# CycloneBoy/pdf_table

Hardware: AMD Instinct MI355X
Metric: pages/s (higher is better)
Workload: dtype bf16

## Files before the change

### pdf_table_amd/csrc/lore_kernels.hip

```cpp
#include <stdio.h>
#include <stdlib.h>

#include "common.h"

namespace PT_FMT_NS {

typedef __attribute__((ext_vector_type(4))) uint32_t u32x4;
typedef __attribute__((ext_vector_type(2))) uint32_t u32x2;

namespace {

__device__ __forceinline__ float bf2f(uint32_t b) { return a16_to_f32(b); }
__device__ __forceinline__ uint32_t f2bf(float f) { return f32_to_a16(f); }

__device__ __forceinline__ void load8(const bf16_t* p, int lo_off, int split, float* v) {
  const u32x4 h = *reinterpret_cast<const u32x4*>(p);
  const uint32_t hw[4] = {h.x, h.y, h.z, h.w};
#pragma unroll
  for (int k = 0; k < 8; ++k) v[k] = bf2f((k & 1) ? (hw[k >> 1] >> 16) : (hw[k >> 1] & 0xFFFFu));
  if (split) {
    const u32x4 l = *reinterpret_cast<const u32x4*>(p + lo_off);
    const uint32_t lw[4] = {l.x, l.y, l.z, l.w};
#pragma unroll
    for (int k = 0; k < 8; ++k) v[k] += bf2f((k & 1) ? (lw[k >> 1] >> 16) : (lw[k >> 1] & 0xFFFFu));
// ... 241 lines not shown
  const int y = i / W, x = i - y * W;
  const pt_tsr_table tb = tabs[t];
  auto sat = [](double v) { return (long long)fmin(fmax(rint(v), -2147483648.0), 2147483647.0); };
  const long long adelta = sat(tb.minv[0] * x * 1024.0), bdelta = sat(tb.minv[3] * x * 1024.0);
  const long long X0 = sat((tb.minv[1] * y + tb.minv[2]) * 1024.0) + 16, Y0 = sat((tb.minv[4] * y + tb.minv[5]) * 1024.0) + 16;
  const long long X = (X0 + adelta) >> 5, Y = (Y0 + bdelta) >> 5;
  long long sx = X >> 5, sy = Y >> 5;
  sx = sx < -32768 ? -32768 : (sx > 32767 ? 32767 : sx);
  sy = sy < -32768 ? -32768 : (sy > 32767 ? 32767 : sy);
  const int ax = (int)(X & 31), ay = (int)(Y & 31);
  const int wt[4] = {(32 - ay) * (32 - ax) * 32, (32 - ay) * ax * 32, ay * (32 - ax) * 32, ay * ax * 32};
  int acc[3] = {0, 0, 0};
  const uint8_t* pg = pages + (size_t)tb.page * ph * pw * 3;
#pragma unroll
  for (int k = 0; k < 4; ++k) {
    const long long yy = sy + (k >> 1), xx = sx + (k & 1);
    if (yy < 0 || yy >= tb.crop_h || xx < 0 || xx >= tb.crop_w) continue;
    const long long py = tb.y0 + yy, px = tb.x0 + xx;
    if (py < 0 || py >= ph || px < 0 || px >= pw) continue;
    const uint8_t* s = pg + ((size_t)py * pw + px) * 3;
    acc[0] += s[0] * wt[k]; acc[1] += s[1] * wt[k]; acc[2] += s[2] * wt[k];
  }
  float v[3];
#pragma unroll
  for (int c = 0; c < 3; ++c) {
    const int sc = bgr ? 2 - c : c;
    int u = (acc[sc] + (1 << 14)) >> 15;
    u = u < 0 ? 0 : (u > 255 ? 255 : u);
    v[c] = lut[c * 256 + u];
  }
  bf16_t* o = out + ((size_t)t * H * W + i) * (split ? 8 : 4);
  uint32_t hb[3];
#pragma unroll
  for (int c = 0; c < 3; ++c) { hb[c] = f2bf(v[c]); o[c] = (bf16_t)hb[c]; }
  o[3] = 0;
  if (split) {
#pragma unroll
    for (int c = 0; c < 3; ++c) o[4 + c] = (bf16_t)f2bf(v[c] - bf2f(hb[c]));
    o[7] = 0;
  }
}

typedef __attribute__((ext_vector_type(8))) __bf16 dbf16x8;
typedef __attribute__((ext_vector_type(16))) float df32x16;
typedef __attribute__((ext_vector_type(2))) float df2;
__device__ __forceinline__ uint32_t pack_df2(df2 v) { return pack_a16x2(v.x, v.y); }
__device__ __forceinline__ df2 unpack_df2(uint32_t pk) { return df2{a16lo_f32(pk), a16hi_f32(pk)}; }

template <int SPLIT, int NB>
__global__ __launch_bounds__(256, (SPLIT || NB > 64) ? 2 : 4) void dcn_fused_kernel(const bf16_t* __restrict__ x, const float* __restrict__ om,
                                                            const bf16_t* __restrict__ w, const float* __restrict__ bias,
                                                            bf16_t* __restrict__ out, long long npix, int H, int W, int C,
                                                            int N, int relu) {
#pragma clang fp contract(fast)
  a16_kernel_enter();
  constexpr int ROW = 80;
  constexpr int NP = SPLIT ? 2 : 1;
  constexpr int NT = NB / 32;
  __shared__ __attribute__((aligned(16))) char s_a[NP][128 * ROW];
  __shared__ __attribute__((aligned(16))) char s_w[NP][NB * ROW];
  const int tid = threadIdx.x, lane = tid & 63, wave = tid >> 6;
  const int lx = lane & 31, q = lane >> 5;
  const long long p0 = (long long)blockIdx.x * 128;
  const int n0 = blockIdx.y * NB;
  const int cs = SPLIT ? 2 * C : C;
  const int nslice = C >> 5, nk = 9 * nslice;
  const int gp = tid & 127, gh = tid >> 7;
  long long pix = p0 + gp;
  const bool live = pix < npix;
  if (!live) pix = npix - 1;
  const int xw = (int)(pix % W), yh = (int)((pix / W) % H);
  const bf16_t* xb = x + (size_t)(pix / ((long long)W * H)) * H * W * cs;
  const float* omp = om + pix * 32;
  constexpr int WPIECES = NB * 4 / 256;
  const bf16_t* wbase = w + (size_t)(n0 >> 6) * (SPLIT ? 3 : 1) * nk * (64 * 32);

  df32x16 acc[NT];
#pragma unroll
  for (int t = 0; t < NT; ++t)
#pragma unroll
    for (int r = 0; r < 16; ++r) acc[t][r] = 0.f;

  int coff[4];
  float cwt[4], mask = 0.f;
  u32x4 rc[NP][4][2];
  u32x4 rw[NP][WPIECES];

  auto geometry = [&](int tap) {
    const float off_h = omp[2 * tap], off_w = omp[2 * tap + 1];
    mask = 1.f / (1.f + expf(-omp[18 + tap]));
    const float h_im = (float)(yh - 1 + tap / 3) + off_h;
    const float w_im = (float)(xw - 1 + tap % 3) + off_w;
#pragma unroll
    for (int k = 0; k < 4; ++k) { coff[k] = -1; cwt[k] = 0.f; }
    if (h_im > -1.f && w_im > -1.f && h_im < (float)H && w_im < (float)W) {
      const float hf = floorf(h_im), wf = floorf(w_im);
      const int h_low = (int)hf, w_low = (int)wf, h_high = h_low + 1, w_high = w_low + 1;
      const float lh = h_im - hf, lw = w_im - wf, hh = 1.f - lh, hw = 1.f - lw;
      cwt[0] = hh * hw; cwt[1] = hh * lw; cwt[2] = lh * hw; cwt[3] = lh * lw;
      if (h_low >= 0 && w_low >= 0) coff[0] = (h_low * W + w_low) * cs;
      if (h_low >= 0 && w_high <= W - 1) coff[1] = (h_low * W + w_high) * cs;
      if (h_high <= H - 1 && w_low >= 0) coff[2] = (h_high * W + w_low) * cs;
      if (h_high <= H - 1 && w_high <= W - 1) coff[3] = (h_high * W + w_high) * cs;
    }
  };
  auto prefetch = [&](int kc) {
    const int tap = kc / nslice, sl = kc - tap * nslice;
    if (sl == 0) geometry(tap);
    const int ch = sl * 32 + gh * 16;
#pragma unroll
    for (int k = 0; k < 4; ++k) {
      const u32x4 z = {0u, 0u, 0u, 0u};
#pragma unroll
      for (int pp = 0; pp < NP; ++pp) {
        rc[pp][k][0] = z; rc[pp][k][1] = z;
        if (coff[k] >= 0) {
          const bf16_t* sp = xb + coff[k] + ch + pp * C;
          rc[pp][k][0] = *reinterpret_cast<const u32x4*>(sp);
          rc[pp][k][1] = *reinterpret_cast<const u32x4*>(sp + 8);
        }
      }
    }
#pragma unroll
    for (int j = 0; j < WPIECES; ++j) {
      const int idx = tid + j * 256;
      const int row = idx >> 2, part = idx & 3;
      const bf16_t* wc = wbase + (size_t)(row >> 6) * (SPLIT ? 3 : 1) * nk * (64 * 32) + (size_t)kc * (64 * 32) + (row & 63) * 32 + part * 8;
      rw[0][j] = *reinterpret_cast<const u32x4*>(wc);
      if (SPLIT) rw[1][j] = *reinterpret_cast<const u32x4*>(wc + (size_t)2 * nk * (64 * 32));
    }
  };
  auto commit = [&]() {
    const df2 w0 = {cwt[0], cwt[0]}, w1 = {cwt[1], cwt[1]}, w2 = {cwt[2], cwt[2]}, w3 = {cwt[3], cwt[3]}, mk = {mask, mask};
    uint32_t oh[8], ol[8];
#pragma unroll
    for (int hgrp = 0; hgrp < 2; ++hgrp) {
#pragma unroll
      for (int e2 = 0; e2 < 4; ++e2) {
        df2 c[4];
#pragma unroll
        for (int k = 0; k < 4; ++k) {
          const uint32_t u = e2 == 0 ? rc[0][k][hgrp].x : e2 == 1 ? rc[0][k][hgrp].y : e2 == 2 ? rc[0][k][hgrp].z : rc[0][k][hgrp].w;
          c[k] = df2{a16lo_f32(u), a16hi_f32(u)};
          if (SPLIT) {
            const uint32_t ul = e2 == 0 ? rc[NP - 1][k][hgrp].x : e2 == 1 ? rc[NP - 1][k][hgrp].y
                                : e2 == 2 ? rc[NP - 1][k][hgrp].z : rc[NP - 1][k][hgrp].w;
            c[k] += df2{a16lo_f32(ul), a16hi_f32(ul)};
          }
        }
        df2 v = w0 * c[0];
        v = w1 * c[1] + v;
        v = w2 * c[2] + v;
        v = w3 * c[3] + v;
        v = v * mk;
        const uint32_t hb = pack_df2(v);
        oh[hgrp * 4 + e2] = hb;
        if (SPLIT) ol[hgrp * 4 + e2] = pack_df2(v - unpack_df2(hb));
      }
    }
    char* ap = s_a[0] + gp * ROW + gh * 32;
    *reinterpret_cast<u32x4*>(ap) = u32x4{oh[0], oh[1], oh[2], oh[3]};
    *reinterpret_cast<u32x4*>(ap + 16) = u32x4{oh[4], oh[5], oh[6], oh[7]};
    if (SPLIT) {
      char* al = s_a[NP - 1] + gp * ROW + gh * 32;
      *reinterpret_cast<u32x4*>(al) = u32x4{ol[0], ol[1], ol[2], ol[3]};
      *reinterpret_cast<u32x4*>(al + 16) = u32x4{ol[4], ol[5], ol[6], ol[7]};
    }
#pragma unroll
    for (int j = 0; j < WPIECES; ++j) {
      const int idx = tid + j * 256;
#pragma unroll
      for (int pp = 0; pp < NP; ++pp) *reinterpret_cast<u32x4*>(s_w[pp] + (idx >> 2) * ROW + (idx & 3) * 16) = rw[pp][j];
    }
  };

  const char* a_rd = s_a[0] + (wave * 32 + lx) * ROW + q * 16;
  const char* b_rd = s_w[0] + lx * ROW + q * 16;
  constexpr int A_PLANE = 128 * ROW, W_PLANE = NB * ROW;
  prefetch(0);
  for (int kc = 0; kc < nk; ++kc) {
    __syncthreads();
    commit();
    __syncthreads();
    if (kc + 1 < nk) prefetch(kc + 1);
#pragma unroll
    for (int kk = 0; kk < 2; ++kk) {
      const dbf16x8 ah = *reinterpret_cast<const dbf16x8*>(a_rd + kk * 32);
      dbf16x8 al;
      if (SPLIT) al = *reinterpret_cast<const dbf16x8*>(a_rd + A_PLANE + kk * 32);
#pragma unroll
      for (int t = 0; t < NT; ++t) {
        const dbf16x8 bh = *reinterpret_cast<const dbf16x8*>(b_rd + t * 32 * ROW + kk * 32);
        acc[t] = mfma_32x32x16_a16(ah, bh, acc[t]);
        if (SPLIT) {
          acc[t] = mfma_32x32x16_a16(al, bh, acc[t]);
          const dbf16x8 bl = *reinterpret_cast<const dbf16x8*>(b_rd + W_PLANE + t * 32 * ROW + kk * 32);
          acc[t] = mfma_32x32x16_a16(ah, bl, acc[t]);
        }
      }
    }
  }
  const int ocs = SPLIT ? 2 * N : N;
#pragma unroll
  for (int t = 0; t < NT; ++t) {
    const int n = n0 + t * 32 + lx;
    const float bv = bias[n];
#pragma unroll
    for (int r = 0; r < 16; ++r) {
      const long long op = p0 + wave * 32 + (r & 3) + 8 * (r >> 2) + 4 * q;
      if (op >= npix) continue;
      float v = acc[t][r] + bv;
      if (relu) v = fmaxf(v, 0.f);
      const uint32_t hb = f2bf(v);
      out[(size_t)op * ocs + n] = (bf16_t)hb;
      if (SPLIT) out[(size_t)op * ocs + N + n] = (bf16_t)f2bf(v - bf2f(hb));
    }
  }
}

#ifndef PT_DCN_ABL
#define PT_DCN_ABL 0
#endif
template <int NB, int NTHR, int SPLIT = 0, int EARLY = 0, int OMF = 0>
__global__ __launch_bounds__(NTHR, SPLIT ? (NB == 128 ? 1 : 2) : NTHR / 128) void dcn_fused64_kernel(const bf16_t* __restrict__ x, const float* __restrict__ om,
                                                              const bf16_t* __restrict__ w, const float* __restrict__ bias,
                                                              bf16_t* __restrict__ out, long long npix, int H, int W,
                                                              int C, int N, int relu, const bf16_t* __restrict__ omw = nullptr,
                                                              const float* __restrict__ omb = nullptr) {
#pragma clang fp contract(fast)
  a16_kernel_enter();
  constexpr int ROW = 144;
  constexpr int IT = 1024 / NTHR;
  constexpr int PSTEP = NTHR / 8;
  constexpr int WP = NB * 8 / NTHR;
  constexpr int NT = NB * 8 / NTHR;
  constexpr int NP = SPLIT ? 2 : 1;
  __shared__ __attribute__((aligned(16))) unsigned s_goff[128 * 9][4];
  __shared__ __attribute__((aligned(16))) float s_gwt[128 * 9][4];
  __shared__ __attribute__((aligned(16))) char s_ab[NP * (128 * ROW + NB * ROW)];
  static_assert(128 * ROW + NB * ROW >= 128 * 28 * 4, "operand images must cover the staged offset/mask rows");
  constexpr int A_PLANE = 128 * ROW, W_PLANE = NB * ROW;
  char* s_a = s_ab;
  char* s_w = s_ab + NP * A_PLANE;
  float* s_om = reinterpret_cast<float*>(s_ab);
  const int tid = threadIdx.x, lane = tid & 63, wave = tid >> 6;
  const int lx = lane & 31, q = lane >> 5;
  const int tiles_x = (W + 15) >> 4, tiles_y = (H + 7) >> 3;
  int Lb = blockIdx.x;
  const int nblk = blockIdx.y;
  const int tx0 = (Lb % tiles_x) * 16;
  Lb /= tiles_x;
  const int ty0 = (Lb % tiles_y) * 8;
  const long long img0 = (long long)(Lb / tiles_y) * H * W;
  auto locate = [&](int pl, int& y, int& xq) -> bool {
    y = ty0 + (pl >> 4);
    xq = tx0 + (pl & 15);
    const bool ok = y < H && xq < W;
    y = y < H ? y : H - 1;
    xq = xq < W ? xq : W - 1;
    return ok;
  };
  const int n0 = nblk * NB;
  const int nss = C >> 6, nst = 9 * nss, nk = 9 * (C >> 5);
  const int cs = SPLIT ? 2 * C : C;
  const int piece = tid & 7, prow = tid >> 3;
  const char* xmap = reinterpret_cast<const char*>(x + (size_t)img0 * cs);
  if constexpr (OMF) {
    constexpr int HP = 180, HROW = 80;
    constexpr int HIT = (HP * 4 + NTHR - 1) / NTHR;
    constexpr int NG = NTHR / 256;
    static_assert(sizeof(s_goff) >= HP * HROW && sizeof(s_gwt) >= HP * HROW, "a halo buffer must fit each table's space");
    char* s_h = reinterpret_cast<char*>(&s_goff[0][0]);
    char* s_h2 = reinterpret_cast<char*>(&s_gwt[0][0]);
    const int nch = (SPLIT ? 3 : 1) * (C >> 5);
    const int grp = wave >> 2, mt_o = wave & 3;
    const int t_lo = NG == 2 ? (grp ? 5 : 0) : 0, t_hi = NG == 2 ? (grp ? 9 : 5) : 9;
    u32x4 hreg[HIT];
    auto halo_load = [&](int kc) {
      int c0 = kc * 32;
      if (SPLIT && kc >= 2 * (C >> 5)) c0 -= 2 * C;
#pragma unroll
      for (int j = 0; j < HIT; ++j) {
        const int i = tid + j * NTHR;
        const int hp = i >> 2, hy = hp / 18, hx = hp - hy * 18;
        const int y = ty0 - 1 + hy, xq = tx0 - 1 + hx;
        u32x4 v = {0u, 0u, 0u, 0u};
        if (i < HP * 4 && (unsigned)y < (unsigned)H && (unsigned)xq < (unsigned)W)
          v = *reinterpret_cast<const u32x4*>(xmap + ((size_t)y * W + xq) * (2 * cs) + (size_t)c0 * 2 + (i & 3) * 16);
        hreg[j] = v;
      }
    };
    auto halo_store = [&](char* buf) {
#pragma unroll
      for (int j = 0; j < HIT; ++j) {
        const int i = tid + j * NTHR;
        if (i < HP * 4) *reinterpret_cast<u32x4*>(buf + (i >> 2) * HROW + (i & 3) * 16) = hreg[j];
      }
    };
    df32x16 oacc;
#pragma unroll
    for (int r = 0; r < 16; ++r) oacc[r] = 0.f;
    const int pl_o = mt_o * 32 + lx;
    const int a_off = ((pl_o >> 4) * 18 + (pl_o & 15)) * HROW + q * 16;
    const bf16_t* wl = omw + (size_t)lx * 32 + q * 8;
    constexpr int NTAP = NG == 2 ? 5 : 9;
    dbf16x8 bfr[NTAP][2];
    auto load_b = [&](int kc, int t) {
      const bf16_t* wt = wl + ((size_t)kc * 9 + (t_lo + t)) * 2048;
      bfr[t][0] = *reinterpret_cast<const dbf16x8*>(wt);
      bfr[t][1] = *reinterpret_cast<const dbf16x8*>(wt + 16);
    };
    halo_load(0);
#pragma unroll
    for (int t = 0; t < NTAP; ++t)
      if (t_lo + t < t_hi) load_b(0, t);
    for (int kc = 0; kc < nch; ++kc) {
      char* buf = (kc & 1) ? s_h2 : s_h;
      halo_store(buf);
      if (kc + 1 < nch) halo_load(kc + 1);
      __syncthreads();
#pragma unroll
      for (int t = 0; t < NTAP; ++t) {
        const int tap = t_lo + t;
        if (tap < t_hi) {
          const char* ap = buf + a_off + ((tap / 3) * 18 + (tap % 3)) * HROW;
          const dbf16x8 a0 = *reinterpret_cast<const dbf16x8*>(ap);
          const dbf16x8 a1 = *reinterpret_cast<const dbf16x8*>(ap + 32);
          oacc = mfma_32x32x16_a16(a0, bfr[t][0], oacc);
          oacc = mfma_32x32x16_a16(a1, bfr[t][1], oacc);
          if (kc + 1 < nch) load_b(kc + 1, t);
        }
      }
    }
    if (wave < 4 && lx < 27) {
      const float bo = omb[lx];
#pragma unroll
      for (int r = 0; r < 16; ++r) s_om[(mt_o * 32 + (r & 3) + 8 * (r >> 2) + 4 * q) * 28 + lx] = oacc[r] + bo;
    }
    if (NG == 2) {
      __syncthreads();
      if (wave >= 4 && lx < 27) {
#pragma unroll
        for (int r = 0; r < 16; ++r) s_om[(mt_o * 32 + (r & 3) + 8 * (r >> 2) + 4 * q) * 28 + lx] += oacc[r];
      }
    }
  } else {
    for (int i = tid; i < 128 * 7; i += NTHR) {
      int y, xq;
      locate(i / 7, y, xq);
      const long long pix = img0 + (long long)y * W + xq;
      *reinterpret_cast<float4*>(s_om + (i / 7) * 28 + (i % 7) * 4) = *reinterpret_cast<const float4*>(om + pix * 32 + (i % 7) * 4);
    }
  }
  __syncthreads();
  for (int i = tid; i < 128 * 9; i += NTHR) {
    const int pl = i / 9, tap = i - pl * 9;
    int yh, xw;
    locate(pl, yh, xw);
    const float* o = s_om + pl * 28;
    const float off_h = o[2 * tap], off_w = o[2 * tap + 1];
    const float gm = 1.f / (1.f + expf(-o[18 + tap]));
    const float h_im = (float)(yh - 1 + tap / 3) + off_h;
    const float w_im = (float)(xw - 1 + tap % 3) + off_w;
    unsigned co[4] = {0u, 0u, 0u, 0u};
    float cw[4] = {0.f, 0.f, 0.f, 0.f};
    if (h_im > -1.f && w_im > -1.f && h_im < (float)H && w_im < (float)W) {
      const float hf = floorf(h_im), wf = floorf(w_im);
      const int h_low = (int)hf, w_low = (int)wf, h_high = h_low + 1, w_high = w_low + 1;
      const float lh = h_im - hf, lw = w_im - wf, hh = 1.f - lh, hw = 1.f - lw;
      if (h_low >= 0 && w_low >= 0) { co[0] = (unsigned)(h_low * W + w_low) * (unsigned)(2 * cs); cw[0] = hh * hw * gm; }
      if (h_low >= 0 && w_high <= W - 1) { co[1] = (unsigned)(h_low * W + w_high) * (unsigned)(2 * cs); cw[1] = hh * lw * gm; }
      if (h_high <= H - 1 && w_low >= 0) { co[2] = (unsigned)(h_high * W + w_low) * (unsigned)(2 * cs); cw[2] = lh * hw * gm; }
      if (h_high <= H - 1 && w_high <= W - 1) { co[3] = (unsigned)(h_high * W + w_high) * (unsigned)(2 * cs); cw[3] = lh * lw * gm; }
    }
    *reinterpret_cast<uint4*>(s_goff[i]) = make_uint4(co[0], co[1], co[2], co[3]);
    *reinterpret_cast<float4*>(s_gwt[i]) = make_float4(cw[0], cw[1], cw[2], cw[3]);
  }
  __syncthreads();
  const bf16_t* wbase = w + (size_t)(n0 >> 6) * (SPLIT ? 3 : 1) * nk * (64 * 32);

  df32x16 acc[NT];
#pragma unroll
  for (int t = 0; t < NT; ++t)
#pragma unroll
    for (int r = 0; r < 16; ++r) acc[t][r] = 0.f;

  unsigned coff[IT][4];
  float cwt[IT][4];
  u32x4 rc[IT][4], rcl[SPLIT ? IT : 1][4];
  u32x4 rw[WP], rwl[SPLIT ? WP : 1];

  auto geometry = [&](int tap) {
#pragma unroll
    for (int j = 0; j < IT; ++j) {
      const int gi = (prow + PSTEP * j) * 9 + tap;
      const uint4 o = *reinterpret_cast<const uint4*>(s_goff[gi]);
      const float4 wv = *reinterpret_cast<const float4*>(s_gwt[gi]);
      coff[j][0] = o.x + piece * 16; coff[j][1] = o.y + piece * 16; coff[j][2] = o.z + piece * 16; coff[j][3] = o.w + piece * 16;
      cwt[j][0] = wv.x; cwt[j][1] = wv.y; cwt[j][2] = wv.z; cwt[j][3] = wv.w;
    }
  };
  auto prefetch = [&](int st) {
    const int tap = st / nss, ss = st - tap * nss;
    if (ss == 0) geometry(tap);
    const char* xs = xmap + ss * 128;
#pragma unroll
    for (int j = 0; j < IT; ++j)
#pragma unroll
      for (int k = 0; k < 4; ++k) {
#if PT_DCN_ABL == 1
        rc[j][k] = u32x4{coff[j][k], 0u, 0u, 0u};
#else
        rc[j][k] = *reinterpret_cast<const u32x4*>(xs + coff[j][k]);
#endif
        if (SPLIT) rcl[j][k] = *reinterpret_cast<const u32x4*>(xs + 2 * C + coff[j][k]);
      }
    const int kc = tap * (C >> 5) + 2 * ss;
#pragma unroll
    for (int j = 0; j < WP; ++j) {
      const int idx = tid + j * NTHR;
      const int row = idx >> 3, pc = idx & 7;
      const bf16_t* wsrc = wbase + (size_t)(row >> 6) * (SPLIT ? 3 : 1) * nk * (64 * 32) + (size_t)(kc + (pc >> 2)) * (64 * 32) +
                           (row & 63) * 32 + (pc & 3) * 8;
      rw[j] = *reinterpret_cast<const u32x4*>(wsrc);
      if (SPLIT) rwl[j] = *reinterpret_cast<const u32x4*>(wsrc + (size_t)2 * nk * (64 * 32));
    }
  };
  auto commit = [&]() {
#pragma unroll
    for (int j = 0; j < IT; ++j) {
#if PT_DCN_ABL == 2
      *reinterpret_cast<u32x4*>(s_a + (prow + PSTEP * j) * ROW + piece * 16) = rc[j][0] ^ rc[j][1] ^ rc[j][2] ^ rc[j][3];
      continue;
#endif
      const df2 w0 = {cwt[j][0], cwt[j][0]}, w1 = {cwt[j][1], cwt[j][1]}, w2 = {cwt[j][2], cwt[j][2]},
                w3 = {cwt[j][3], cwt[j][3]};
      uint32_t o[4], ol[4];
#pragma unroll
      for (int e2 = 0; e2 < 4; ++e2) {
        if constexpr (PT_A16_HAS_MIX_BLEND && !SPLIT) {
          o[e2] = a16_blend4(rc[j][0][e2], rc[j][1][e2], rc[j][2][e2], rc[j][3][e2], cwt[j][0], cwt[j][1], cwt[j][2], cwt[j][3]);
          continue;
        }
        df2 c[4];
#pragma unroll
        for (int k = 0; k < 4; ++k) {
          const uint32_t u = e2 == 0 ? rc[j][k].x : e2 == 1 ? rc[j][k].y : e2 == 2 ? rc[j][k].z : rc[j][k].w;
          c[k] = df2{a16lo_f32(u), a16hi_f32(u)};
          if (SPLIT) {
            const uint32_t ul = e2 == 0 ? rcl[j][k].x : e2 == 1 ? rcl[j][k].y : e2 == 2 ? rcl[j][k].z : rcl[j][k].w;
            c[k] += df2{a16lo_f32(ul), a16hi_f32(ul)};
          }
        }
        df2 v = w0 * c[0];
        v = w1 * c[1] + v;
        v = w2 * c[2] + v;
        v = w3 * c[3] + v;
        const uint32_t hb = pack_df2(v);
        o[e2] = hb;
        if (SPLIT) ol[e2] = pack_df2(v - unpack_df2(hb));
      }
      *reinterpret_cast<u32x4*>(s_a + (prow + PSTEP * j) * ROW + piece * 16) = u32x4{o[0], o[1], o[2], o[3]};
      if (SPLIT) *reinterpret_cast<u32x4*>(s_a + A_PLANE + (prow + PSTEP * j) * ROW + piece * 16) = u32x4{ol[0], ol[1], ol[2], ol[3]};
    }
#pragma unroll
    for (int j = 0; j < WP; ++j) {
      const int idx = tid + j * NTHR;
      *reinterpret_cast<u32x4*>(s_w + (idx >> 3) * ROW + (idx & 7) * 16) = rw[j];
      if (SPLIT) *reinterpret_cast<u32x4*>(s_w + W_PLANE + (idx >> 3) * ROW + (idx & 7) * 16) = rwl[j];
    }
  };

  const int mt = wave & 3, ct0 = (wave >> 2) * NT;
  const char* a_rd = s_a + (mt * 32 + lx) * ROW + q * 16;
  const char* b_rd = s_w + (ct0 * 32 + lx) * ROW + q * 16;
  auto product = [&]() {
#pragma unroll
    for (int kk = 0; kk < 4; ++kk) {
      const dbf16x8 a = *reinterpret_cast<const dbf16x8*>(a_rd + kk * 32);
      dbf16x8 al;
      if (SPLIT) al = *reinterpret_cast<const dbf16x8*>(a_rd + A_PLANE + kk * 32);
#pragma unroll
      for (int t = 0; t < NT; ++t) {
        const dbf16x8 b = *reinterpret_cast<const dbf16x8*>(b_rd + t * 32 * ROW + kk * 32);
#if PT_DCN_ABL == 3
        if (kk == 0 && t == 0)
#endif
        acc[t] = mfma_32x32x16_a16(b, a, acc[t]);
        if (SPLIT) {
          acc[t] = mfma_32x32x16_a16(b, al, acc[t]);
          const dbf16x8 bl = *reinterpret_cast<const dbf16x8*>(b_rd + W_PLANE + t * 32 * ROW + kk * 32);
          acc[t] = mfma_32x32x16_a16(bl, a, acc[t]);
        }
      }
    }
  };
  if constexpr (EARLY && !SPLIT) {
    prefetch(0);
    for (int st = 0; st < nst; ++st) {
      const bool more = st + 1 < nst;
      const int tap_n = (st + 1) / nss, ss_n = (st + 1) - tap_n * nss;
      const char* xs_n = xmap + ss_n * 128;
      __syncthreads();
#pragma unroll
      for (int j = 0; j < IT; ++j) {
        const df2 w0 = {cwt[j][0], cwt[j][0]}, w1 = {cwt[j][1], cwt[j][1]}, w2 = {cwt[j][2], cwt[j][2]}, w3 = {cwt[j][3], cwt[j][3]};
        uint32_t o[4];
#pragma unroll
        for (int e2 = 0; e2 < 4; ++e2) {
          if constexpr (PT_A16_HAS_MIX_BLEND) {
            o[e2] = a16_blend4(rc[j][0][e2], rc[j][1][e2], rc[j][2][e2], rc[j][3][e2], cwt[j][0], cwt[j][1], cwt[j][2], cwt[j][3]);
            continue;
          }
          df2 c[4];
#pragma unroll
          for (int k = 0; k < 4; ++k) {
            const uint32_t u = e2 == 0 ? rc[j][k].x : e2 == 1 ? rc[j][k].y : e2 == 2 ? rc[j][k].z : rc[j][k].w;
            c[k] = df2{a16lo_f32(u), a16hi_f32(u)};
          }
          df2 v = w0 * c[0];
          v = w1 * c[1] + v;
          v = w2 * c[2] + v;
          v = w3 * c[3] + v;
          o[e2] = pack_df2(v);
        }
        *reinterpret_cast<u32x4*>(s_a + (prow + PSTEP * j) * ROW + piece * 16) = u32x4{o[0], o[1], o[2], o[3]};
        if (more) {
          if (ss_n == 0) {
            const int gi = (prow + PSTEP * j) * 9 + tap_n;
            const uint4 og = *reinterpret_cast<const uint4*>(s_goff[gi]);
            const float4 wv = *reinterpret_cast<const float4*>(s_gwt[gi]);
            coff[j][0] = og.x + piece * 16; coff[j][1] = og.y + piece * 16; coff[j][2] = og.z + piece * 16; coff[j][3] = og.w + piece * 16;
            cwt[j][0] = wv.x; cwt[j][1] = wv.y; cwt[j][2] = wv.z; cwt[j][3] = wv.w;
          }
#pragma unroll
          for (int k = 0; k < 4; ++k) rc[j][k] = *reinterpret_cast<const u32x4*>(xs_n + coff[j][k]);
        }
      }
#pragma unroll
      for (int j = 0; j < WP; ++j) {
        const int idx = tid + j * NTHR;
        *reinterpret_cast<u32x4*>(s_w + (idx >> 3) * ROW + (idx & 7) * 16) = rw[j];
      }
      if (more) {
        const int kc = tap_n * (C >> 5) + 2 * ss_n;
#pragma unroll
        for (int j = 0; j < WP; ++j) {
          const int idx = tid + j * NTHR;
          const int row = idx >> 3, pc = idx & 7;
          rw[j] = *reinterpret_cast<const u32x4*>(wbase + (size_t)(row >> 6) * nk * (64 * 32) + (size_t)(kc + (pc >> 2)) * (64 * 32) + (row & 63) * 32 + (pc & 3) * 8);
        }
      }
      __syncthreads();
      product();
    }
  } else {
    prefetch(0);
    for (int st = 0; st < nst; ++st) {
      __syncthreads();
      commit();
      __syncthreads();
      if (st + 1 < nst) prefetch(st + 1);
      product();
    }
  }
  int y, xq;
  if (locate(mt * 32 + lx, y, xq)) {
    bf16_t* op = out + (size_t)(img0 + (long long)y * W + xq) * (SPLIT ? 2 * N : N) + n0 + ct0 * 32;
#pragma unroll
    for (int t = 0; t < NT; ++t)
#pragma unroll
      for (int rg = 0; rg < 4; ++rg) {
        const int ch = t * 32 + 8 * rg + 4 * q;
        const float4 bs = *reinterpret_cast<const float4*>(bias + n0 + ct0 * 32 + ch);
        float v[4] = {acc[t][rg * 4 + 0] + bs.x, acc[t][rg * 4 + 1] + bs.y, acc[t][rg * 4 + 2] + bs.z, acc[t][rg * 4 + 3] + bs.w};
        if (relu) {
#pragma unroll
          for (int j = 0; j < 4; ++j) v[j] = fmaxf(v[j], 0.f);
        }
        const uint32_t h0 = f2bf(v[0]), h1 = f2bf(v[1]), h2 = f2bf(v[2]), h3 = f2bf(v[3]);
        *reinterpret_cast<uint2*>(op + ch) = make_uint2(h0 | (h1 << 16), h2 | (h3 << 16));
        if (SPLIT)
          *reinterpret_cast<uint2*>(op + N + ch) = make_uint2(f2bf(v[0] - bf2f(h0)) | (f2bf(v[1] - bf2f(h1)) << 16),
                                                               f2bf(v[2] - bf2f(h2)) | (f2bf(v[3] - bf2f(h3)) << 16));
      }
  }
}

#ifndef PT_DCN_MABL
#define PT_DCN_MABL 0
#endif
#ifndef PT_DCN_RING64
#define PT_DCN_RING64 4
#endif
template <int NB, int RING>
struct DcnMfmaSmem {
  static constexpr int BYTES = 128 * 9 * 24 + 2 * NB * 128 + 8 * RING * 1024;
};
template <int NB, int RING>
__global__ __launch_bounds__(512, (NB == 64 && RING == 4) ? 2 : 1) void dcn_mfma_kernel(const bf16_t* __restrict__ x, const float* __restrict__ om,
                                                                            const bf16_t* __restrict__ w, const float* __restrict__ bias,
                                                                            bf16_t* __restrict__ out, long long npix, int H, int W, int C,
                                                                            int N, int relu) {
#pragma clang fp contract(fast)
  a16_kernel_enter();
  static_assert(RING == 4 || RING == 8, "ring slots must divide the eight steps of a stage");
  constexpr int NT = NB / 32;
  constexpr int WP = NB / 64;
  constexpr int D = RING - 1;
  constexpr int GOFF_BYTES = 128 * 9 * 16, GW_BYTES = 128 * 9 * 8, W_BYTES = NB * 128;
  extern __shared__ __attribute__((aligned(16))) char smem[];
  char* s_goff = smem;
  char* s_gw = smem + GOFF_BYTES;
  char* s_w = s_gw + GW_BYTES;
  char* s_ring = s_w + 2 * W_BYTES;
  float* s_om = reinterpret_cast<float*>(s_ring);
  static_assert(8 * RING * 1024 >= 128 * 28 * 4, "ring must cover the staged offset / mask rows");
  const int tid = threadIdx.x, lane = tid & 63, wave = tid >> 6;
  const int lx = lane & 31, q = lane >> 5;
  const int pt = wave & 3, hh = wave >> 2;
  const int tiles_x = (W + 15) >> 4, tiles_y = (H + 7) >> 3;
  int Lb = blockIdx.x;
  const int tx0 = (Lb % tiles_x) * 16;
  Lb /= tiles_x;
  const int ty0 = (Lb % tiles_y) * 8;
  const long long img0 = (long long)(Lb / tiles_y) * H * W;
  auto locate = [&](int pl, int& y, int& xq) -> bool {
    y = ty0 + (pl >> 4);
    xq = tx0 + (pl & 15);
    const bool ok = y < H && xq < W;
    y = y < H ? y : H - 1;
    xq = xq < W ? xq : W - 1;
    return ok;
  };
  const int n0 = blockIdx.y * NB;
  const int nss = C >> 6, nst = 9 * nss, nk = 9 * (C >> 5);
// ... 989 lines not shown
```

Baseline: 779.5.

## Stage offset-conv weights through shared memory instead of per-wave register prefetch

Offset-conv weights for each channel chunk are now loaded cooperatively by the whole block into registers, stored into a padded LDS region that reuses the operand-image buffer, and read from LDS by each wave for the MFMA taps. Before, every wave fetched its own B fragments from global memory into a large per-tap register array. The aim is to cut redundant global loads and register pressure. In exchange it adds an extra barrier per chunk and a trailing one, and uses more LDS traffic.

```diff
diff --git a/pdf_table_amd/csrc/lore_kernels.hip b/pdf_table_amd/csrc/lore_kernels.hip
--- a/pdf_table_amd/csrc/lore_kernels.hip
+++ b/pdf_table_amd/csrc/lore_kernels.hip
@@ -567,36 +567,49 @@
     for (int r = 0; r < 16; ++r) oacc[r] = 0.f;
     const int pl_o = mt_o * 32 + lx;
     const int a_off = ((pl_o >> 4) * 18 + (pl_o & 15)) * HROW + q * 16;
-    const bf16_t* wl = omw + (size_t)lx * 32 + q * 8;
-    constexpr int NTAP = NG == 2 ? 5 : 9;
-    dbf16x8 bfr[NTAP][2];
-    auto load_b = [&](int kc, int t) {
-      const bf16_t* wt = wl + ((size_t)kc * 9 + (t_lo + t)) * 2048;
-      bfr[t][0] = *reinterpret_cast<const dbf16x8*>(wt);
-      bfr[t][1] = *reinterpret_cast<const dbf16x8*>(wt + 16);
+    constexpr int OWROW = 80, OWTAP = 32 * OWROW, OWP = 9 * 32 * 4;
+    constexpr int OWIT = (OWP + NTHR - 1) / NTHR;
+    static_assert(sizeof(s_ab) >= 9 * OWTAP, "the operand images must hold a chunk's staged offset-conv weights");
+    char* s_ow = s_ab;
+    u32x4 owreg[OWIT];
+    auto ow_load = [&](int kc) {
+#pragma unroll
+      for (int j = 0; j < OWIT; ++j) {
+        const int i = tid + j * NTHR;
+        if (i < OWP) owreg[j] = *reinterpret_cast<const u32x4*>(omw + ((size_t)kc * 9 + (i >> 7)) * 2048 + ((i >> 2) & 31) * 32 + (i & 3) * 8);
+      }
     };
+    auto ow_store = [&]() {
+#pragma unroll
+      for (int j = 0; j < OWIT; ++j) {
+        const int i = tid + j * NTHR;
+        if (i < OWP) *reinterpret_cast<u32x4*>(s_ow + (i >> 7) * OWTAP + ((i >> 2) & 31) * OWROW + (i & 3) * 16) = owreg[j];
+      }
+    };
+    const char* b_o = s_ow + lx * OWROW + q * 16;
     halo_load(0);
-#pragma unroll
-    for (int t = 0; t < NTAP; ++t)
-      if (t_lo + t < t_hi) load_b(0, t);
+    ow_load(0);
     for (int kc = 0; kc < nch; ++kc) {
       char* buf = (kc & 1) ? s_h2 : s_h;
+      if (kc > 0) __syncthreads();
       halo_store(buf);
-      if (kc + 1 < nch) halo_load(kc + 1);
+      ow_store();
+      if (kc + 1 < nch) {
+        halo_load(kc + 1);
+        ow_load(kc + 1);
+      }
       __syncthreads();
-#pragma unroll
-      for (int t = 0; t < NTAP; ++t) {
-        const int tap = t_lo + t;
-        if (tap < t_hi) {
-          const char* ap = buf + a_off + ((tap / 3) * 18 + (tap % 3)) * HROW;
-          const dbf16x8 a0 = *reinterpret_cast<const dbf16x8*>(ap);
-          const dbf16x8 a1 = *reinterpret_cast<const dbf16x8*>(ap + 32);
-          oacc = mfma_32x32x16_a16(a0, bfr[t][0], oacc);
-          oacc = mfma_32x32x16_a16(a1, bfr[t][1], oacc);
-          if (kc + 1 < nch) load_b(kc + 1, t);
-        }
-      }
-    }
+      for (int tap = t_lo; tap < t_hi; ++tap) {
+        const char* ap = buf + a_off + ((tap / 3) * 18 + (tap % 3)) * HROW;
+        const dbf16x8 a0 = *reinterpret_cast<const dbf16x8*>(ap);
+        const dbf16x8 a1 = *reinterpret_cast<const dbf16x8*>(ap + 32);
+        const dbf16x8 b0 = *reinterpret_cast<const dbf16x8*>(b_o + tap * OWTAP);
+        const dbf16x8 b1 = *reinterpret_cast<const dbf16x8*>(b_o + tap * OWTAP + 32);
+        oacc = mfma_32x32x16_a16(a0, b0, oacc);
+        oacc = mfma_32x32x16_a16(a1, b1, oacc);
+      }
+    }
+    __syncthreads();
     if (wave < 4 && lx < 27) {
       const float bo = omb[lx];
 #pragma unroll
```

Result: no change. 784.0, median of 6 (+0.6%).
